# Isaac-McPadden/Farkle_II

Measured on AMD Instinct MI355X. Metric: simulated games/sec (whole node) at k=2, fixed strategy-grid size, higher is better.
Workload: dtype int32; 1 GPU; BASELINE configs[1]: k=2, 64-strategy grid, 10^7 games per GPU per step, root_seed 42, counts-only tallies; k=2, root_seed=42, parallelism=shuffle-range split x1, device=AMD Radeon Graphics, arch=gfx950:sramecc+:xnack-, compute_units=256, clock_mhz=2400

## Files before the change

farkle_ii_amd/backend.py:

```python
from __future__ import annotations

import ctypes as C
import os
import subprocess
from pathlib import Path

import numpy as np

from .strategies import STRATEGY_DTYPE

PKG_DIR = Path(__file__).resolve().parent
LIB_PATH = Path(os.environ.get("FARKLE_HIP_LIB", PKG_DIR / "libfarkle_hip.so"))
SRC_DIR = PKG_DIR / "csrc"
HIPCC = os.environ.get("HIPCC", "/opt/rocm/bin/hipcc")

COORD_DTYPE = np.dtype(
    [("purpose", "<u4"), ("pad", "<u4"), ("root_seed", "<u8"), ("k", "<u8"), ("shuffle_index", "<u8"),
     ("pair_id", "<u8"), ("order", "<u8"), ("game_index", "<u8"), ("seat_index", "<u8"), ("replicate_index", "<u8")]
)
OVERRIDE_DTYPE = np.dtype(
    [("root_seed", "<u8"), ("a", "<u8"), ("b", "<u8"), ("k_or_order", "<u4"), ("max_rounds", "<u4")]
)
SEAT_DTYPE = np.dtype(
    [("score", "<i4"), ("strategy", "<i4"), ("farkles", "<u2"), ("rolls", "<u2"), ("n_turns", "<u2"),
# ... 6 lines not shown
)
EVENT_DTYPE = np.dtype(
    [("dice", "<u4"), ("turn_score", "<i4"), ("points", "<u2"), ("round", "<u2"), ("seat", "u1"), ("used_left", "u1"),
     ("discards", "u1"), ("flags", "u1")]
)
TALLY_COLS = 26
LAG_COLS = 11
SEAT_STAT_COLS = 31
SEAT_RATIO_COLS = 4
SEAT_STAT_NAMES = ("exposures", "completed_exposures", "safety_limit_exposures", "wins", "final_score_sum", "final_score_square_sum",
                   "n_turns_sum", "n_turns_square_sum", "turn_round_mismatch_count", "turn_minus_rounds_sum",
                   "turn_minus_rounds_square_sum") + tuple(
    f"{name}_{kind}" for name in ("rank", "loss_margin", "rolls", "farkles", "highest_turn", "hot_dice", "smart_five_uses",
                                   "n_smart_five_dice", "smart_one_uses", "n_smart_one_dice") for kind in ("sum", "square_sum"))
COL_WINS, COL_ATTEMPTED, COL_COMPLETED, COL_SAFETY, COL_SUMS, COL_SQ_SUMS = 0, 1, 2, 3, 4, 15

FK_ERR_ROLL_LIMIT, FK_ERR_ARG, FK_ERR_COUNTER_OVERFLOW, FK_ERR_HIP, FK_ERR_NO_DEVICE, FK_ERR_COMM = -1, -2, -3, -4, -5, -6
COMM_ID_BYTES = 128


def row_dtype(k: int) -> np.dtype:
    return np.dtype([("n_rounds", "<u2"), ("status", "u1"), ("winner_seat", "i1"), ("seats", SEAT_DTYPE, (k,))])


class _DeviceInfo(C.Structure):
    _fields_ = [("name", C.c_char * 64), ("arch", C.c_char * 32), ("compute_units", C.c_int32), ("clock_mhz", C.c_int32),
                ("wavefront_size", C.c_int32), ("lds_bytes_per_cu", C.c_int32), ("hbm_bytes", C.c_uint64)]


class _Timing(C.Structure):
    _fields_ = [("perm_ms", C.c_float), ("seed_ms", C.c_float), ("play_ms", C.c_float), ("total_ms", C.c_float),
                ("play_launches", C.c_int32), ("play_block", C.c_int32), ("play_grid", C.c_int32),
                ("play_lds_bytes", C.c_int32), ("games", C.c_int64), ("prefetched_chunks", C.c_int32), ("play_clock_mhz", C.c_int32),
                ("play_block_end_p50_ms", C.c_float), ("play_block_end_max_ms", C.c_float), ("play_mixed_flags", C.c_int32)]


class FarkleHipError(RuntimeError):

    def __init__(self, code: int, message: str):
        super().__init__(message)
        self.code = code


def hip_sources() -> list[Path]:
    return [SRC_DIR / "farkle_hip.hip"]


VARIANTS = {"detour": ["-DFK_FORCE_DETOUR=4"]}


def library_path(variant: str | None = None) -> Path:
    return LIB_PATH if not variant else LIB_PATH.with_name(f"libfarkle_hip_{variant}.so")


def build_library(force: bool = False, verbose: bool = False, variant: str | None = None) -> Path:
    out = library_path(variant)
    deps = hip_sources() + [SRC_DIR / "fk_device.h", SRC_DIR / "fk_kernels.h", SRC_DIR / "fk_play_hc.h", SRC_DIR / "fk_shard_writer.h", SRC_DIR / "fk_perm_wave.h", SRC_DIR / "fk_row_columns_seats.h", SRC_DIR / "fk_matchups.h", SRC_DIR / "fk_game_stats.h", SRC_DIR / "fk_rare_events.h", SRC_DIR / "fk_bootstrap.h", SRC_DIR / "fk_root_stability.h", SRC_DIR / "fk_seat_analysis.h", SRC_DIR / "fk_trace.h", PKG_DIR.parent / "include" / "farkle_hip.h"]
    if out.exists() and not force and all(out.stat().st_mtime >= d.stat().st_mtime for d in deps):
        return out
    cmd = [HIPCC, "--offload-arch=gfx950", "-O3", "-std=c++17", "-fPIC", "-shared", *(VARIANTS[variant] if variant else []), "-o", str(out),
           *[str(s) for s in hip_sources()]]
    res = subprocess.run(cmd, capture_output=True, text=True)
    if verbose or res.returncode != 0:
        print(" ".join(cmd))
        print(res.stdout, res.stderr)
    if res.returncode != 0:
        raise RuntimeError(f"hipcc failed ({res.returncode}): {res.stderr[-2000:]}")
    return out


_EXPORTS = ["fk_init", "fk_destroy", "fk_last_error", "fk_get_device_info", "fk_get_timing", "fk_set_option",
            "fk_tournament_run", "fk_tournament_run_stats", "fk_tournament_run_all_player", "fk_tournament_run_game_stats", "fk_tournament_run_rare_events", "fk_tournament_run_lags", "fk_tournament_run_matchups", "fk_matchup_reduce", "fk_tournament_hint_next", "fk_play_games", "fk_h2h_run", "fk_h2h_run_blocks", "fk_coordinate_seeds", "fk_debug_score", "fk_debug_should_continue",
            "fk_debug_dice", "fk_debug_dice_state", "fk_debug_dice_keys", "fk_comm_unique_id", "fk_comm_init", "fk_reduce_tally", "fk_comm_destroy", "fk_tally_resident_reduce", "fk_comm_ranks", "fk_host_alloc", "fk_host_free", "fk_game_seeds",
            "fk_tournament_run_columns", "fk_row_columns_bytes", "fk_write_row_shards", "fk_debug_sha256", "fk_get_option", "fk_debug_deadline_handshake", "fk_debug_hold_memory", "fk_rows_wait", "fk_tournament_run_columns_seeds",
            "fk_last_play_instance", "fk_debug_bounded_draws", "fk_performance_bootstrap", "fk_root_stability_bootstrap", "fk_tournament_run_seat_counts", "fk_trace_games"]
_libs: dict = {}


def load_library(variant: str | None = None) -> C.CDLL:
    if variant not in _libs:
        path = library_path(variant)
        if not path.exists():
            raise FileNotFoundError(
                f"{path} is missing: build it with `python -c 'import __graft_entry__ as g; g.build()'` "
                "(there is no CPU fallback for the simulation path)")
        lib = C.CDLL(str(path))
        for name in _EXPORTS:
            getattr(lib, name)
        lib.fk_last_error.restype = C.c_char_p
        lib.fk_last_error.argtypes = [C.c_void_p]
        lib.fk_last_play_instance.restype = C.c_char_p
        lib.fk_last_play_instance.argtypes = [C.c_void_p]
        lib.fk_destroy.restype = None
# ... 691 lines not shown
```

farkle_ii_amd/csrc/farkle_hip.hip:

```cpp
#include "fk_kernels.h"
#include "fk_shard_writer.h"
#include "fk_perm_wave.h"
#include "fk_row_columns_seats.h"
#include "fk_matchups.h"
#include "fk_game_stats.h"
#include "fk_rare_events.h"
#include "fk_bootstrap.h"
#include "fk_root_stability.h"
#include "fk_seat_analysis.h"
#include "fk_trace.h"

#include <dlfcn.h>
#include <rccl/rccl.h>
#include <unistd.h>

#include <algorithm>
#include <atomic>
#include <chrono>
#include <cmath>
#include <memory>
#include <mutex>
#include <sys/mman.h>
#include <unordered_map>
#include <thread>
// ... 94 lines not shown
    const SeatReq *seats;
};

struct fk_ctx {
    int device = 0;
    hipStream_t stream = nullptr;
    hipStream_t prep_stream = nullptr;
    ChunkSet sets[2];
    int cur = 0;
    uint64_t table_epoch = 0;
    bool hint_valid = false;
    uint64_t hint_begin = 0, hint_end = 0;
    int32_t hint_state = 0, pipeline = 1;
    hipDeviceProp_t prop{};
    std::string err;
    fk_timing timing{};
    std::string play_instance;
    hipEvent_t ev[8] = {nullptr, nullptr, nullptr, nullptr, nullptr, nullptr, nullptr, nullptr};
    int32_t *err_host = nullptr;
    hipEvent_t main_idle = nullptr;
    struct PendingTimer {
        float *acc;
        hipEvent_t a, b;
    };
    std::vector<PendingTimer> pending;
    DevBuf strat, recs, rec0, tally, rows, ov, seatlist, coords, inv, slow, score_lut, discard_lut, block_out, stats, ratios, digest,
        dbg[6];
    std::vector<uint2> strat_host;
    int32_t longest_first = 1;
    int32_t blocks_per_cu = 0;
    int32_t max_waves = 6;
    int32_t lean = -1;
    int32_t gs = -1;
    int32_t uniform_flags_opt = -1;
    uint32_t table_flags = 0;
    uint32_t table_mixed_flags = 0xff00u;
    int64_t chunk_bytes = (int64_t)48 << 30;
    int32_t workspace_percent = 80;
    int64_t chunk_limit = 0;
    int64_t last_budget = 0;
    bool oom = false;
    std::vector<void *> hog;
    int32_t oom_replays = 0;
    int32_t batch_threshold = 0;
    int32_t use_lds_tally = -1;
    int32_t block = 0;
    int32_t hc = -1;
    int32_t hc_waves = 5;
    int32_t hc_block = 256;
    int32_t hc_tables = 1;
    int32_t hc_inc_regs = 1;
    int32_t hc_cl = -1;
    DevBuf lds_tables;
    DevBuf cold;
    int32_t clock_stamps = 0;
    DevBuf clk;
    int clk_grid = 0;
    DevBuf lag_v, lag_out, lag_lags, lag_edge, lag_tmp;
    DevBuf m_ids, m_dig, m_seat, m_rnd;
    DevBuf mr[36];
    uint64_t matchup_sort_mask = ~0ull;
    DevBuf g_rec, g_out;
    int64_t game_stats_window = 0;
    DevBuf r_sec, r_out, r_blk, r_base, r_head, r_seats;
    DevBuf sa_counts, sa[16];
    DevBuf tr[8];
// ... 615 lines not shown
    HIPCHK(c, hipGetLastError());
    return FK_OK;
}

size_t game_workspace_bytes(int32_t k, bool full_state, bool recs, bool rows) {
    return (size_t)k * ((full_state ? STATE_DW * 4 : 18) + 16) + 8 + (recs ? REC_DW * 4 + 4 : 0) +
           (rows ? sizeof(fk_row_hdr) + sizeof(fk_seat) * (size_t)k : 0);
}

int launch_play_stage(fk_ctx *c, const SeedArgs &sa, PlayArgs &pa, const LaunchPlan &plan, bool want_state, bool want_rec0, bool want_recs) {
    ChunkSet &cs = CSET(c);
    int rc;
    if (want_rec0) {
        rc = ensure(c, c->rec0, (size_t)sa.n_games * 4);
        if (rc) return rc;
    }
    if (want_recs) {
        rc = ensure(c, c->recs, (size_t)sa.n_games * REC_DW * 4);
        if (rc) return rc;
    }
    pa.sched = sa.sched;
    pa.seat_idx = sa.seat_idx;
    pa.state = sa.state;
    pa.state_dw = sa.state_dw;
    pa.inc = sa.inc;
    pa.rec0 = want_rec0 ? static_cast<uint32_t *>(c->rec0.p) : nullptr;
    pa.recs = want_recs ? static_cast<uint32_t *>(c->recs.p) : nullptr;
    pa.gs_out = (want_state && !plan.gs) ? 1u : 0u;
    pa.ticket = static_cast<uint32_t *>(cs.misc.p);
    pa.err = reinterpret_cast<int32_t *>(static_cast<uint8_t *>(cs.misc.p) + 16);
    const int auto_thr = sa.k >= 11 ? 16 : sa.k >= 9 ? 12 : 8;
    pa.batch_threshold = (uint32_t)std::max(1, std::min(64, c->batch_threshold > 0 ? c->batch_threshold : auto_thr));
    pa.use_lds_tally = plan.lds_tally ? 1u : 0u;
    pa.clk = nullptr;
    c->clk_grid = 0;
    if (c->clock_stamps) {
        const size_t bytes = (size_t)std::max(plan.grid, 1) * 4 * sizeof(unsigned long long);
        rc = ensure(c, c->clk, bytes);
        if (rc) return rc;
        HIPCHK(c, hipMemsetAsync(c->clk.p, 0, bytes, c->stream));
        pa.clk = static_cast<unsigned long long *>(c->clk.p);
    }
    {
        Timer t(c, &c->timing.play_ms, SLOT_PLAY);
        LaunchPlan lp = plan;
        lp.mixed_flags = (c->uniform_flags_opt != 0) ? c->table_mixed_flags : 0xff00u;
        pa.uflags = c->table_flags;
        hipError_t e = launch_play(lp, pa, c->stream);
        t.stop();
        HIPCHK(c, e);
        c->play_instance = lp.instance ? lp.instance : "";
        c->timing.play_grid = lp.launched_grid;
        c->timing.play_mixed_flags = lp.mixed_flags == MIXED_NONE ? (int32_t)MIXED_NONE
                                     : (lp.mixed_flags & ~MIXED_RB_FAV) == 0u ? (int32_t)MIXED_RB_FAV : (int32_t)MIXED_ALL;
        if (pa.clk) c->clk_grid = lp.launched_grid;
    }
    c->timing.play_launches += 1;
    c->timing.play_block = plan.block;
    c->timing.play_lds_bytes = (int32_t)plan.lds;
    c->timing.games += sa.n_games;
    return FK_OK;
}

int finish_timers(fk_ctx *c) {
    HIPCHK(c, collect_timers(c));
    if (c->clk_grid > 0) {
// ... 1 lines not shown
        HIPCHK(c, hipMemcpy(h.data(), c->clk.p, h.size() * sizeof(unsigned long long), hipMemcpyDeviceToHost));
        std::vector<double> mhz, ends;
        unsigned long long first = ~0ull;
        for (int b = 0; b < c->clk_grid; ++b) {
            const unsigned long long t0 = h[(size_t)b * 4], r0 = h[(size_t)b * 4 + 1], t1 = h[(size_t)b * 4 + 2], r1 = h[(size_t)b * 4 + 3];
            if (r1 > r0 && t1 > t0) {
                mhz.push_back(100.0 * (double)(t1 - t0) / (double)(r1 - r0));
                ends.push_back((double)r1);
                first = r0 < first ? r0 : first;
            }
        }
        if (!mhz.empty()) {
            std::nth_element(mhz.begin(), mhz.begin() + (std::ptrdiff_t)(mhz.size() / 2), mhz.end());
            c->timing.play_clock_mhz = (int32_t)(mhz[mhz.size() / 2] + 0.5);
            std::nth_element(ends.begin(), ends.begin() + (std::ptrdiff_t)(ends.size() / 2), ends.end());
            c->timing.play_block_end_p50_ms = (float)((ends[ends.size() / 2] - (double)first) * 1e-5);
            c->timing.play_block_end_max_ms = (float)((*std::max_element(ends.begin(), ends.end()) - (double)first) * 1e-5);
        }
        c->clk_grid = 0;
    }
    ChunkSet &cs = CSET(c);
    float ms = 0.f;
    if (hipEventElapsedTime(&ms, cs.ev[0], cs.ev[1]) == hipSuccess) c->timing.perm_ms += ms;
    if (cs.side) {
        c->timing.prefetched_chunks += 1;
    } else if (hipEventElapsedTime(&ms, cs.ev[2], cs.ev[3]) == hipSuccess) {
        c->timing.seed_ms += ms;
    }
    return FK_OK;
}

int finish_play(fk_ctx *c, const PlayArgs &pa, int64_t game_base, const char *what) {
    const int rc_dev = check_device_error(c, pa.err, game_base, what);
    const int rc = finish_timers(c);
    return rc_dev ? rc_dev : rc;
}

int run_chunk(fk_ctx *c, const SeedArgs &sa_in, PlayArgs pa, const LaunchPlan &plan, bool want_state, bool want_rec0, bool want_recs,
              int64_t game_base, const char *what) {
    SeedArgs sa = sa_in;
    ChunkSet &cs = CSET(c);
    cs.prepared = false;
    cs.side = false;
    HIPCHK(c, hipStreamWaitEvent(c->stream, cs.ready, 0));
    (void)hipEventRecord(cs.ev[0], c->stream);
    (void)hipEventRecord(cs.ev[1], c->stream);
    int rc = seed_stage(c, c->cur, c->stream, sa, plan.gs || want_state, true);
    if (rc) return rc;
    rc = launch_play_stage(c, sa, pa, plan, want_state, want_rec0, want_recs);
    if (rc) return rc;
    return finish_play(c, pa, game_base, what);
}

int prep_tournament_chunk(fk_ctx *c, int si, hipStream_t st_seed, const ChunkDesc &d, SeedArgs &sa) {
    ChunkSet &cs = c->sets[si];
    cs.prepared = false;
    hipStream_t st = c->stream;
    HIPCHK(c, hipStreamWaitEvent(st, cs.ready, 0));
    const int32_t S = (int32_t)d.S;
    const uint32_t n_sh = d.n_sh, slots = d.slots, gps = d.S / d.k;
    const uint32_t perm_blocks = (n_sh + slots - 1u) / slots;
    const SeedPool perm_prefix = seed_prefix(101u , d.root, (uint64_t)d.k);
    int rc = ensure(c, cs.perm, (size_t)perm_blocks * S * slots * 2);
    if (rc) return rc;
    (void)hipEventRecord(cs.ev[0], st);
    {
// ... 462 lines not shown
}

int fk_set_option(fk_ctx *c, const char *name, int64_t value) {
    if (!c || !name) return FK_ERR_ARG;
    std::string n(name);
    if (n == "chunk_bytes") c->chunk_bytes = std::max<int64_t>(value, 1 << 20);
    else if (n == "workspace_percent") c->workspace_percent = (int32_t)std::min<int64_t>(std::max<int64_t>(value, 1), 100000);
    else if (n == "comm_timeout_ms") {
        c->comm_timeout_ms = (int32_t)std::min<int64_t>(std::max<int64_t>(value, 0), 86400000);
        c->comm_timeout_set = true;
    }
    else if (n == "batch_threshold") c->batch_threshold = (int32_t)value;
    else if (n == "use_lds_tally") c->use_lds_tally = (int32_t)value;
    else if (n == "longest_first") c->longest_first = (int32_t)value;
    else if (n == "blocks_per_cu") c->blocks_per_cu = (int32_t)value;
    else if (n == "max_waves") c->max_waves = (int32_t)std::min<int64_t>(std::max<int64_t>(value, 1), 8);
    else if (n == "lean") c->lean = (int32_t)value;
    else if (n == "state_store") c->gs = (int32_t)value;
    else if (n == "rows_chunk_games") c->rows_chunk_games = std::max<int64_t>(value, 1);
    else if (n == "rows_async") c->rows_async = value != 0;
    else if (n == "resident_tally") {
        c->resident = value != 0;
        c->acc_n = 0;
    } else if (n == "hot_cold") {
        if (value != -1 && value != 0) return fail(c, FK_ERR_ARG, "hot_cold is -1 (auto: four and more seats) or 0 (never)");
        c->hc = (int32_t)value;
    }
    else if (n == "clock_stamps") c->clock_stamps = value != 0;
    else if (n == "perm_split") c->perm_split = (int32_t)value;
    else if (n == "perm_draw_wave") c->perm_draw_wave = (int32_t)value;
    else if (n == "columns_by_seat") c->columns_by_seat = (int32_t)value;
    else if (n == "pipeline") c->pipeline = (int32_t)value;
    else if (n == "uniform_flags") c->uniform_flags_opt = (int32_t)value;
    else if (n == "matchup_sort_key_mask") c->matchup_sort_mask = (uint64_t)value;
    else if (n == "game_stats_window") c->game_stats_window = std::max<int64_t>(value, 0);
    else if (n == "bootstrap_block") c->bootstrap_block = std::max<int64_t>(value, 0);
    else if (n == "block") {
        if (value != 0 && value != 64 && value != 128 && value != 256 && value != 512 && value != 768 && value != 1024)
            return fail(c, FK_ERR_ARG, "block must be 0, 64, 128, 256, 512, 768 (lean records only) or 1024");
        c->block = (int32_t)value;
    } else return fail(c, FK_ERR_ARG, "unknown option %s", name);
    return FK_OK;
}

int fk_rows_wait(fk_ctx *c, int32_t slot) {
    if (!c || slot < 0 || slot >= FK_ROWS_EVENTS) return FK_ERR_ARG;
    HIPCHK(c, hipSetDevice(c->device));
    HIPCHK(c, hipEventSynchronize(c->ev_call_copy[slot]));
    return FK_OK;
}

size_t fk_row_columns_bytes(int32_t k, int32_t games_per_shuffle) {
    return (k < 1 || games_per_shuffle < 1) ? 0 : fksw::shard_image_bytes(k, games_per_shuffle);
}

int fk_write_row_shards(const fk_shard_job *job, int64_t *byte_length, uint8_t *sha256, uint8_t *sidecar_sha256, char *error, size_t error_len) {
    auto say = [&](const std::string &m) {
        if (error && error_len) std::snprintf(error, error_len, "%s", m.c_str());
        return FK_ERR_ARG;
    };
    if (!job || !byte_length || !sha256) return say("job, byte_length and sha256 are required");
    if (!job->shuffle_index || !job->shuffle_seed || !job->batch_id || !job->game_seed || !job->columns || !job->directory || !job->footer_head ||
        !job->footer_kv || !job->footer_orders || !job->leaf_type || !job->leaf_paths)
        return say("a required field of the shard job is null");
    if ((job->side_body != nullptr) != (job->side_full != nullptr) || (job->side_body && (!job->side_directory || !sidecar_sha256)))
        return say("the sidecar template needs body, full, directory and a sidecar_sha256 output");
// ... 452 lines not shown
        pa.seat_strategy = nullptr;
        pa.tally = static_cast<unsigned long long *>(c->tally.p);
        pa.ov = static_cast<const DevOverride *>(c->ov.p);
        pa.n_ov = (uint32_t)dov.size();
        pa.mode = MODE_PERM;
        pa.n_games = n_games;
        pa.gps = gps;
        pa.n_sh = n_sh;
        pa.k = (uint32_t)k;
        pa.S = (uint32_t)S;
        pa.target50 = ceil_div50(target_score);
        pa.beat50 = floor_div50(target_score);
        pa.max_rounds = (uint32_t)max_rounds;
        pa.cold = static_cast<uint4 *>(c->cold.p);
        pa.lds_tables = static_cast<const uint8_t *>(c->lds_tables.p);

        HIPCHK(c, hipEventRecord(c->main_idle, c->stream));
        if (c->pipeline) {
            ChunkDesc next{};
            bool have_next = false;
            if (done + chunk_sh < n_sh_total) {
                next = describe(sh0 + n_sh, (uint32_t)std::min<uint64_t>(chunk_sh, n_sh_total - done - chunk_sh), state_dw);
                have_next = true;
            } else if (hinted) {
                next = describe(hint_begin, (uint32_t)std::min<uint64_t>(chunk_sh, hint_end - hint_begin), hint_dw);
                have_next = true;
            }
            if (have_next) {
                if ((rc = prep_tournament_chunk(c, c->cur ^ 1, c->prep_stream, next, c->sets[c->cur ^ 1].sa))) return rc;
            }
        }
        if (wait_ready) HIPCHK(c, hipStreamWaitEvent(c->stream, c->sets[c->cur].ready, 0));
        if ((rc = launch_play_stage(c, sa, pa, plan, want_state, want_recs || sq != nullptr, want_recs))) return rc;
        const bool defer_check = done + chunk_sh >= n_sh_total && !rows && c->err_host;
        if (defer_check) {
            HIPCHK(c, hipMemcpyAsync(c->err_host, pa.err, 2 * sizeof(int32_t), hipMemcpyDeviceToHost, c->stream));
            deferred = true;
            deferred_base = (int64_t)done * gps;
        } else {
            if ((rc = finish_play(c, pa, (int64_t)done * gps, "tournament"))) return rc;
        }
        const bool scheduled = c->longest_first != 0;
        if (want_state && scheduled) {
            if ((rc = ensure(c, c->inv, (size_t)n_games * 4))) return rc;
            hipLaunchKernelGGL(fk_invert_sched_kernel, dim3((n_games + 255u) / 256u), dim3(256), 0, c->stream,
                               static_cast<const uint32_t *>(CSET(c).order.p), n_games, static_cast<uint32_t *>(c->inv.p));
        }
        if (seat_stats || gst || sq) {
            rc = ensure(c, CSET(c).draws, (size_t)perm_blocks * S * slots * 2);
            if (rc) return rc;
            const uint32_t cells = perm_blocks * (uint32_t)S * slots;
            hipLaunchKernelGGL(fk_invert_perm_kernel, dim3((cells + 255u) / 256u), dim3(256), 0, c->stream,
                               static_cast<const uint16_t *>(CSET(c).perm.p), (uint32_t)S, slots, n_sh, static_cast<uint16_t *>(CSET(c).draws.p));
        }
        if (gst) {
            unsigned long long *o = static_cast<unsigned long long *>(c->g_out.p);
            const uint32_t rec_grid = std::max<uint32_t>(1u, std::min<uint32_t>((n_games + 255u) / 256u, 2048u));
            hipLaunchKernelGGL(fkg::fk_game_record_kernel, dim3(rec_grid), dim3(256), (size_t)(g_wr + g_wm + fkg::N_COUNTS) * 4, c->stream,
                               static_cast<const uint32_t *>(CSET(c).state.p), static_cast<const uint32_t *>(c->recs.p),
                               scheduled ? static_cast<const uint32_t *>(c->inv.p) : nullptr, n_games, gps, n_sh, (uint32_t)k, gst->rare_target,
                               g_wr, g_wm, static_cast<uint4 *>(c->g_rec.p), o + g_gc, o + g_gr, o + g_gru, g_spill);
            const uint32_t want_seg = std::max<uint32_t>(1u, (2048u + (uint32_t)S - 1u) / (uint32_t)S);
            const uint32_t rows_per_seg = std::max<uint32_t>(256u, (n_sh + want_seg - 1u) / want_seg);
            const uint32_t n_seg = (n_sh + rows_per_seg - 1u) / rows_per_seg;
            hipLaunchKernelGGL(fkg::fk_game_stats_gather_kernel, dim3((uint32_t)S, n_seg), dim3(256), (size_t)(g_wr + 2 * g_wm + fkg::N_COUNTS) * 4,
                               c->stream, static_cast<const uint4 *>(c->g_rec.p), static_cast<const uint16_t *>(CSET(c).draws.p), slots,
                               (uint32_t)S, (uint32_t)k, gps, n_sh, rows_per_seg, g_wr, g_wm, g_rb, g_mb, o + g_sc, o + g_sr, o + g_sru, o + g_ssp,
// ... 1548 lines not shown
```

farkle_ii_amd/csrc/fk_device.h:

```cpp
#pragma once

#include <hip/hip_runtime.h>
#include <stdint.h>

namespace fk {

constexpr uint32_t SS_INIT_A = 0x43b0d7e5u, SS_MULT_A = 0x931e8875u;
constexpr uint32_t SS_INIT_B = 0x8b51f9ddu, SS_MULT_B = 0x58f38dedu;
constexpr uint32_t SS_MIX_L = 0xca01f9ddu, SS_MIX_R = 0x4973f715u;

__host__ __device__ constexpr uint32_t ss_hc(int c) {
    uint32_t h = SS_INIT_A;
    for (int i = 0; i < c; ++i) h *= SS_MULT_A;
    return h;
}

__host__ __device__ inline uint32_t ss_hashmix(uint32_t v, uint32_t &hc) {
    v ^= hc;
    hc *= SS_MULT_A;
    v *= hc;
    v ^= v >> 16;
    return v;
}

// ... 853 lines not shown
}

template <bool LEAN, uint32_t MIXED = 0xffffu>
__host__ __device__ inline bool roll_back_end50w(uint32_t e, uint32_t x, uint32_t n, const Strat50 &sp, uint32_t uniform_bits, bool final_round,
                                                 int32_t stb50, RollRegs &r, bool &overflow) {
    const int32_t score50 = (int32_t)(e & 63u) - (int32_t)((x >> DW_POINTS_SHIFT) & 0xffu);
    const uint32_t used = ((e >> 6) & 7u) - (x >> DW_DICE_SHIFT);
    return roll_back_end50_core<LEAN, MIXED>(score50, used, x & DW_INC, (x >> DW_D1_SHIFT) & DW_INC, n, sp, uniform_bits, final_round, stb50, r, overflow);
}

struct Table2 {
    uint32_t seat, rounds, trigger, final_round, safety;
    int32_t score_to_beat;
};
struct Advance2 {
    bool ended, sw;
};
__host__ __device__ inline Advance2 advance2_table50(bool over, int32_t score, int32_t target50, uint32_t max_rounds, Table2 &t) {
    const bool fr = t.final_round != 0u;
    const bool trig = over & !fr & (score >= target50);
    const bool close = over & !fr & !trig & (t.seat != 0u);
    const bool last = close & (t.rounds >= max_rounds);
    const bool ended = last | (over & fr);
    t.rounds += (close & !last) ? 1u : 0u;
    t.safety = last ? 1u : t.safety;
    t.score_to_beat = trig ? score : t.score_to_beat;
    t.trigger = trig ? t.seat : t.trigger;
    t.final_round = (fr | trig) ? 1u : 0u;
    const bool sw = over & !ended;
    t.seat ^= sw ? 1u : 0u;
    return Advance2{ended, sw};
}

}
```

farkle_ii_amd/csrc/fk_kernels.h:

```cpp
#pragma once

#include "../../include/farkle_hip.h"
#include "fk_device.h"

#include <hip/hip_runtime.h>

using namespace fk;

namespace {

constexpr uint32_t HC_AFTER_6_WORDS = ss_hc(24);
constexpr uint32_t HC_AFTER_12_WORDS = ss_hc(48);
constexpr uint32_t HC_AFTER_14_WORDS = ss_hc(56);

enum : uint32_t { MODE_PERM = 0, MODE_LIST = 1, MODE_BLOCKS = 2 };

enum : uint32_t {
    F_LO0 = 0, F_LO1, F_HI0, F_HI1, F_INC_LO0, F_INC_LO1, F_INC_HI0, F_INC_HI1,
    F_BUF, F_SCORE, F_CA, F_CB, F_CC, F_CD, F_CE, F_SPX, F_SPY, NF
};
constexpr uint32_t CE_HAS_BUF_SHIFT = 17, CE_HAS_SCORED = 1u << 16, CE_HAS_BUF = 1u << CE_HAS_BUF_SHIFT;
static_assert(CE_HAS_SCORED == BE_HAS_SCORED, "fk_device.h's roll back end sets the flag in cE");
constexpr uint32_t CE_IDX_SHIFT = 18;
constexpr uint32_t LEAN_DW = 10;
constexpr int32_t LEAN_MAX_TARGET50 = 64000;

enum : uint32_t { R_LO0 = 0, R_LO1, R_HI0, R_HI1, R_BUF, R_SCORE, R_CA, R_CB, R_CC, R_CD, R_CE, R_IDX, STATE_DW = 12 };

constexpr uint32_t REC_DW = 8, REC_SAFETY = 0x80000000u;

constexpr uint32_t LT_COLS = 24;
constexpr uint32_t TICKET_CHUNK = 64;

struct DevOverride {
    uint32_t game;
    uint32_t max_rounds;
};

// ... 29 lines not shown
};

struct PlayArgs {
    const uint2 *strat;
    const uint32_t *score_lut;
    const uint8_t *discard_lut;
    const uint16_t *perm_T;
    uint32_t perm_slots;
    const int32_t *seat_strategy;
    const uint32_t *game_block;
    uint32_t *state;
    uint32_t state_dw;
    const uint4 *inc;
    const uint16_t *seat_idx;
    const uint32_t *sched;
    unsigned long long *tally;
    uint32_t *rec0;
    uint32_t *recs;
    uint32_t gs_out;
    uint32_t *ticket;
    int32_t *err;
    const DevOverride *ov;
    uint32_t n_ov;
    uint32_t mode;
    uint32_t n_games, gps, n_sh, k, S;
    int32_t target50;
    int32_t beat50;
    uint32_t max_rounds;
    uint32_t batch_threshold;
    uint32_t use_lds_tally;
    uint32_t uflags;
    uint4 *cold;
    const uint8_t *lds_tables;
    unsigned long long *clk;
};

__device__ inline void clock_stamp(unsigned long long *clk, uint32_t which) {
    if (!clk) return;
    unsigned long long *slot = clk + (size_t)blockIdx.x * 4u + 2u * which;
    if (which == 0u) {
        if (threadIdx.x == 0) {
            slot[0] = __builtin_amdgcn_s_memtime();
            slot[1] = __builtin_amdgcn_s_memrealtime();
        }
    } else if ((threadIdx.x & 63u) == 0u) {
        atomicMax(slot, (unsigned long long)__builtin_amdgcn_s_memtime());
        atomicMax(slot + 1, (unsigned long long)__builtin_amdgcn_s_memrealtime());
    }
}

__device__ inline uint32_t lane_id() { return threadIdx.x & 63u; }

__device__ inline uint32_t mbcnt(uint64_t mask) {
    return __builtin_amdgcn_mbcnt_hi((uint32_t)(mask >> 32), __builtin_amdgcn_mbcnt_lo((uint32_t)mask, 0u));
}

__device__ inline Strat unpack_strat(uint2 v) { return Strat{(int32_t)v.x, v.y}; }

__device__ inline uint32_t perm_at(const uint16_t *perm, uint32_t S, uint32_t slots, uint32_t sh, uint32_t e) {
    const uint32_t b = sh / slots, l = sh - b * slots;
    return perm[((size_t)b * S + e) * slots + l];
}

constexpr int PERM_BLOCK = 512, PERM_WAVES = PERM_BLOCK / 64;

__global__ __launch_bounds__(PERM_BLOCK) void fk_perm_kernel(SeedPool prefix, uint64_t shuffle0, uint32_t n_sh, uint32_t S,
// ... 853 lines not shown
                g[0] = make_uint4((uint32_t)rng.lo, (uint32_t)(rng.lo >> 32), (uint32_t)rng.hi, (uint32_t)(rng.hi >> 32));
                g[1] = make_uint4(rng.buf, (uint32_t)score, cA, (cB & 0xffffu) | (own_turns << 16));
                uint32_t *g2 = reinterpret_cast<uint32_t *>(g + 2);
                g2[0] = cC;
                g2[1] = cD;
                g2[2] = (cB >> 16) | (cE & (CE_HAS_SCORED | CE_HAS_BUF));
                advance(score);
                return;
            }
        }
        if (LEAN) {
            rec[0] = make_uint2((uint32_t)rng.lo, (uint32_t)(rng.lo >> 32));
            rec[1] = make_uint2((uint32_t)rng.hi, (uint32_t)(rng.hi >> 32));
            rec[2] = make_uint2(rng.buf, cA);
            rec[3] = make_uint2(cB, cC);
            rec[4] = make_uint2(cD, cE);
        } else {
            L(F_LO0, s) = (uint32_t)rng.lo;
            L(F_LO1, s) = (uint32_t)(rng.lo >> 32);
            L(F_HI0, s) = (uint32_t)rng.hi;
            L(F_HI1, s) = (uint32_t)(rng.hi >> 32);
            L(F_BUF, s) = rng.buf;
            L(F_SCORE, s) = (uint32_t)score;
            L(F_CA, s) = cA;
            L(F_CB, s) = cB;
            L(F_CC, s) = cC;
            L(F_CD, s) = cD;
            L(F_CE, s) = cE;
        }
        if (PK2) advance2(over, score);
        else if (!GS && over) advance(score);
    };

    auto handover = [&](uint64_t waiting) {
        const bool mine = (st == ST_FRESH || st == ST_ENDED);
        if (st == ST_ENDED) finish_game();
        const uint32_t n = (uint32_t)__popcll(waiting);
        const uint32_t avail = pool_end - pool_next;
        uint32_t new_base = 0, new_avail = 0;
        if (avail < n && !exhausted) {
            const uint32_t first = (uint32_t)__builtin_amdgcn_readfirstlane(__ffsll((long long)waiting) - 1);
            uint32_t base = 0;
            if (mine && lane_id() == first) base = atomicAdd(a.ticket, TICKET_CHUNK);
            base = (uint32_t)__builtin_amdgcn_readlane((int)base, (int)first);
            if (base >= a.n_games) {
                exhausted = 1;
            } else {
                new_base = base;
                new_avail = min(TICKET_CHUNK, a.n_games - base);
                if (new_avail < TICKET_CHUNK) exhausted = 1;
            }
        }
        if (mine) {
            const uint32_t rank = mbcnt(waiting);
            uint32_t ticket = 0xffffffffu;
            if (rank < avail) ticket = pool_next + rank;
            else if (rank - avail < new_avail) ticket = new_base + (rank - avail);
            if (ticket != 0xffffffffu) init_game(a.sched ? a.sched[ticket] : ticket, ticket);
            else st = ST_DONE;
        }
        if (n <= avail) {
            pool_next += n;
        } else {
            const uint32_t used_new = min(n - avail, new_avail);
            pool_next = new_base + used_new;
            pool_end = new_base + new_avail;
        }
    };

    auto handover_due = [&](uint64_t waiting, uint64_t active) -> bool {
        return waiting && (!active || (uint32_t)__popcll(waiting) >= a.batch_threshold || exhausted);
    };
    while (true) {
        uint64_t waiting = __ballot(st == ST_FRESH || st == ST_ENDED);
        uint64_t active = __ballot(st == ST_ACTIVE);
        if (!(waiting | active)) break;
        if (handover_due(waiting, active)) {
            handover(waiting);
            continue;
        }
        bool playing = st == ST_ACTIVE;
        do {
            if (playing) roll_step();
            playing = st == ST_ACTIVE;
            waiting = __ballot(st == ST_ENDED);
            active = __ballot(playing);
        } while (active && !handover_due(waiting, active));
    }

    if (a.use_lds_tally) {
        __syncthreads();
        for (uint32_t i = tid; i < a.S * LT_COLS; i += BLOCK) {
            const unsigned long long v = tl[i];
            if (v == 0ull) continue;
            const uint32_t idx = i / LT_COLS, c = i - idx * LT_COLS;
            if (c == LT_COLS - 1u) continue;
            const uint32_t col = (c == 0u) ? 0u : (c == 1u) ? 2u : (c == 2u) ? 3u : (c < 13u) ? (c + 1u) : (c + 2u);
            atomicAdd(&a.tally[(size_t)idx * FK_TALLY_COLS + col], v);
        }
    }
    clock_stamp(a.clk, 1u);
}

#include "fk_play_hc.h"

constexpr uint32_t LAG_WIN_BIT = 0x8000u;

__global__ __launch_bounds__(256) void fk_lag_values_kernel(const uint32_t *recs, const uint16_t *perm_T, uint32_t perm_slots, uint32_t S,
                                                            uint32_t k, uint32_t gps, uint32_t n_games, uint16_t *V) {
    const size_t t = (size_t)blockIdx.x * blockDim.x + threadIdx.x;
    if (t >= (size_t)n_games * k) return;
    const uint32_t id = (uint32_t)(t / k), seat = (uint32_t)(t - (size_t)id * k);
    const uint32_t sh = id / gps, g = id - sh * gps;
    const uint4 q0 = *reinterpret_cast<const uint4 *>(recs + (size_t)id * REC_DW);
    const bool won = !(q0.x & REC_SAFETY) && ((q0.x >> 24) & 0x7fu) == seat;
    const uint32_t idx = perm_at(perm_T, S, perm_slots, sh, g * k + seat);
    V[(size_t)sh * S + idx] = (uint16_t)((q0.z & 0x7fffu) | (won ? LAG_WIN_BIT : 0u));
}

__global__ __launch_bounds__(256) void fk_lag_sums_kernel(const uint16_t *V, uint32_t S, uint32_t valid_from, uint32_t first_row, uint32_t n_rows,
                                                          uint32_t rows_per_seg, const int32_t *lags, uint32_t n_lags, long long *out) {
    const uint32_t s = blockIdx.x * blockDim.x + threadIdx.x;
    if (s >= S) return;
    const uint32_t r0 = first_row + blockIdx.y * rows_per_seg, r1 = min(r0 + rows_per_seg, n_rows);
    for (uint32_t li = 0; li < n_lags; ++li) {
        const uint32_t lag = (uint32_t)lags[li];
        long long n = 0, wx = 0, wy = 0, wxy = 0, rx = 0, ry = 0, rxx = 0, ryy = 0, rxy = 0;
        for (uint32_t r = max(r0, valid_from + lag); r < r1; ++r) {
            const uint32_t later = V[(size_t)r * S + s], earlier = V[(size_t)(r - lag) * S + s];
            const long long a = earlier & 0x7fffu, b = later & 0x7fffu, wa = earlier >> 15, wb = later >> 15;
            n += 1;
            wx += wa, wy += wb, wxy += wa & wb;
            rx += a, ry += b, rxx += a * a, ryy += b * b, rxy += a * b;
// ... 550 lines not shown
```

include/farkle_hip.h:

```cpp
#ifndef FARKLE_HIP_H
#define FARKLE_HIP_H

#include <stddef.h>
#include <stdint.h>

#ifdef __cplusplus
extern "C" {
#endif

enum {
    FK_OK = 0,
    FK_ERR_ROLL_LIMIT = -1,
    FK_ERR_ARG = -2,
    FK_ERR_COUNTER_OVERFLOW = -3,
    FK_ERR_HIP = -4,
    FK_ERR_NO_DEVICE = -5,
    FK_ERR_COMM = -6,
    FK_ERR_IO = -7
};

enum { FK_COMPLETED = 0, FK_SAFETY_LIMIT = 1 };

typedef struct {
    int32_t score_threshold;
// ... 29 lines not shown
    uint32_t purpose;
    uint32_t pad;
    uint64_t root_seed, k, shuffle_index, pair_id, order, game_index, seat_index, replicate_index;
} fk_coord;

#define FK_MAX_PLAYERS 128
#define FK_SEAT_STAT_COLS 31
#define FK_LAG_COLS 11
#define FK_MAX_LAGS 16
#define FK_TALLY_COLS 26

typedef struct {
    char name[64];
    char arch[32];
    int32_t compute_units;
    int32_t clock_mhz;
    int32_t wavefront_size;
    int32_t lds_bytes_per_cu;
    uint64_t hbm_bytes;
} fk_device_info;

typedef struct {
    float perm_ms;
    float seed_ms;
    float play_ms;
    float total_ms;
    int32_t play_launches;
    int32_t play_block, play_grid, play_lds_bytes;
    int64_t games;
    int32_t prefetched_chunks;
    int32_t play_clock_mhz;
    float play_block_end_p50_ms, play_block_end_max_ms;
    int32_t play_mixed_flags;
} fk_timing;

typedef struct fk_ctx fk_ctx;

int fk_init(int device_ordinal, fk_ctx **out);
void fk_destroy(fk_ctx *ctx);
const char *fk_last_error(fk_ctx *ctx);
int fk_get_device_info(fk_ctx *ctx, fk_device_info *out);
int fk_get_timing(fk_ctx *ctx, fk_timing *out);
const char *fk_last_play_instance(fk_ctx *ctx);
int fk_host_alloc(fk_ctx *ctx, size_t bytes, void **out);
int fk_host_free(fk_ctx *ctx, void *p);
int fk_set_option(fk_ctx *ctx, const char *name, int64_t value);
int fk_get_option(fk_ctx *ctx, const char *name, int64_t *value);

int fk_tournament_run(fk_ctx *ctx, const fk_strategy *strategies, int32_t S, int32_t k, uint64_t root_seed,
                      uint64_t shuffle_begin, uint64_t shuffle_end, uint32_t shuffles_per_batch,
                      int32_t target_score, int32_t max_rounds, const fk_override *ov, int32_t n_ov,
                      int64_t *tally, void *rows, int32_t *perms);

int fk_tournament_run_columns(fk_ctx *ctx, const fk_strategy *strategies, int32_t S, int32_t k, uint64_t root_seed,
                              uint64_t shuffle_begin, uint64_t shuffle_end, uint32_t shuffles_per_batch,
                              int32_t target_score, int32_t max_rounds, const fk_override *ov, int32_t n_ov,
                              int64_t *tally, const int32_t *strategy_ids, void *columns);
int fk_tournament_run_columns_seeds(fk_ctx *ctx, const fk_strategy *strategies, int32_t S, int32_t k, uint64_t root_seed,
                                    uint64_t shuffle_begin, uint64_t shuffle_end, uint32_t shuffles_per_batch, int32_t target_score,
                                    int32_t max_rounds, const fk_override *overrides, int32_t n_overrides, int64_t *tally,
                                    const int32_t *strategy_ids, void *columns, uint32_t *shuffle_seeds, uint32_t *game_seeds);
size_t fk_row_columns_bytes(int32_t k, int32_t games_per_shuffle);
int fk_rows_wait(fk_ctx *ctx, int32_t slot);

typedef struct {
    int32_t k, games_per_shuffle, n_shuffles, threads, atomic, rng_purpose_namespace;
// ... 160 lines not shown
```

Baseline: 1.208 billion games/s.

## Add flat k=2 handover path with scalar-register bases and specialized finish

Adds a specialized handover path for two-player games without blocking. Game init and finish use precomputed uniform base addresses held in scalar registers and a feature bitmask, plus a branch-light winner selection (finish2_50). This targets the per-game setup and teardown cost in the wave-level handover loop, which the old path paid through generic init_game/finish_game calls. The new path is on by default and can be turned off with the flat_handover option. A compile-time handover counting variant is also added for profiling; its extra output fields enlarge the timing struct.

```diff
diff --git a/farkle_ii_amd/backend.py b/farkle_ii_amd/backend.py
--- a/farkle_ii_amd/backend.py
+++ b/farkle_ii_amd/backend.py
@@ -62,7 +62,9 @@
     _fields_ = [("perm_ms", C.c_float), ("seed_ms", C.c_float), ("play_ms", C.c_float), ("total_ms", C.c_float),
                 ("play_launches", C.c_int32), ("play_block", C.c_int32), ("play_grid", C.c_int32),
                 ("play_lds_bytes", C.c_int32), ("games", C.c_int64), ("prefetched_chunks", C.c_int32), ("play_clock_mhz", C.c_int32),
-                ("play_block_end_p50_ms", C.c_float), ("play_block_end_max_ms", C.c_float), ("play_mixed_flags", C.c_int32)]
+                ("play_block_end_p50_ms", C.c_float), ("play_block_end_max_ms", C.c_float), ("play_mixed_flags", C.c_int32),
+                ("ho_handovers", C.c_int64), ("ho_lanes_served", C.c_int64), ("ho_trips", C.c_int64),
+                ("ho_waiting_lane_trips", C.c_int64), ("ho_rolling_lane_trips", C.c_int64), ("ho_waves", C.c_int64)]
 
 
 class FarkleHipError(RuntimeError):
@@ -77,6 +79,7 @@
 
 
 VARIANTS = {"detour": ["-DFK_FORCE_DETOUR=4"]}
+TOOL_VARIANTS = {"count": ["-DFK_COUNT_HANDOVER"]}
 
 
 def library_path(variant: str | None = None) -> Path:
@@ -88,7 +91,7 @@
     deps = hip_sources() + [SRC_DIR / "fk_device.h", SRC_DIR / "fk_kernels.h", SRC_DIR / "fk_play_hc.h", SRC_DIR / "fk_shard_writer.h", SRC_DIR / "fk_perm_wave.h", SRC_DIR / "fk_row_columns_seats.h", SRC_DIR / "fk_matchups.h", SRC_DIR / "fk_game_stats.h", SRC_DIR / "fk_rare_events.h", SRC_DIR / "fk_bootstrap.h", SRC_DIR / "fk_root_stability.h", SRC_DIR / "fk_seat_analysis.h", SRC_DIR / "fk_trace.h", PKG_DIR.parent / "include" / "farkle_hip.h"]
     if out.exists() and not force and all(out.stat().st_mtime >= d.stat().st_mtime for d in deps):
         return out
-    cmd = [HIPCC, "--offload-arch=gfx950", "-O3", "-std=c++17", "-fPIC", "-shared", *(VARIANTS[variant] if variant else []), "-o", str(out),
+    cmd = [HIPCC, "--offload-arch=gfx950", "-O3", "-std=c++17", "-fPIC", "-shared", *({**VARIANTS, **TOOL_VARIANTS}[variant] if variant else []), "-o", str(out),
            *[str(s) for s in hip_sources()]]
     res = subprocess.run(cmd, capture_output=True, text=True)
     if verbose or res.returncode != 0:
diff --git a/farkle_ii_amd/csrc/farkle_hip.hip b/farkle_ii_amd/csrc/farkle_hip.hip
--- a/farkle_ii_amd/csrc/farkle_hip.hip
+++ b/farkle_ii_amd/csrc/farkle_hip.hip
@@ -150,6 +150,7 @@
     int32_t max_waves = 6;
     int32_t lean = -1;
     int32_t gs = -1;
+    int32_t flat_handover = 1;
     int32_t uniform_flags_opt = -1;
     uint32_t table_flags = 0;
     uint32_t table_mixed_flags = 0xff00u;
@@ -831,6 +832,12 @@
     const int auto_thr = sa.k >= 11 ? 16 : sa.k >= 9 ? 12 : 8;
     pa.batch_threshold = (uint32_t)std::max(1, std::min(64, c->batch_threshold > 0 ? c->batch_threshold : auto_thr));
     pa.use_lds_tally = plan.lds_tally ? 1u : 0u;
+    pa.no_flat = c->flat_handover ? 0u : 1u;
+#ifdef FK_COUNT_HANDOVER
+    pa.hcount = reinterpret_cast<unsigned long long *>(static_cast<uint8_t *>(cs.misc.p) + 128);
+#else
+    pa.hcount = nullptr;
+#endif
     pa.clk = nullptr;
     c->clk_grid = 0;
     if (c->clock_stamps) {
@@ -898,6 +905,12 @@
 
 int finish_play(fk_ctx *c, const PlayArgs &pa, int64_t game_base, const char *what) {
     const int rc_dev = check_device_error(c, pa.err, game_base, what);
+    if (pa.hcount) {
+        unsigned long long h[6] = {0, 0, 0, 0, 0, 0};
+        HIPCHK(c, hipMemcpy(h, pa.hcount, sizeof(h), hipMemcpyDeviceToHost));
+        c->timing.ho_handovers += (int64_t)h[0], c->timing.ho_lanes_served += (int64_t)h[1], c->timing.ho_trips += (int64_t)h[2];
+        c->timing.ho_waiting_lane_trips += (int64_t)h[3], c->timing.ho_rolling_lane_trips += (int64_t)h[4], c->timing.ho_waves += (int64_t)h[5];
+    }
     const int rc = finish_timers(c);
     return rc_dev ? rc_dev : rc;
 }
@@ -1426,6 +1439,7 @@
     else if (n == "columns_by_seat") c->columns_by_seat = (int32_t)value;
     else if (n == "pipeline") c->pipeline = (int32_t)value;
     else if (n == "uniform_flags") c->uniform_flags_opt = (int32_t)value;
+    else if (n == "flat_handover") c->flat_handover = value != 0 ? 1 : 0;
     else if (n == "matchup_sort_key_mask") c->matchup_sort_mask = (uint64_t)value;
     else if (n == "game_stats_window") c->game_stats_window = std::max<int64_t>(value, 0);
     else if (n == "bootstrap_block") c->bootstrap_block = std::max<int64_t>(value, 0);
@@ -1944,7 +1958,7 @@
         }
         if (wait_ready) HIPCHK(c, hipStreamWaitEvent(c->stream, c->sets[c->cur].ready, 0));
         if ((rc = launch_play_stage(c, sa, pa, plan, want_state, want_recs || sq != nullptr, want_recs))) return rc;
-        const bool defer_check = done + chunk_sh >= n_sh_total && !rows && c->err_host;
+        const bool defer_check = done + chunk_sh >= n_sh_total && !rows && c->err_host && !pa.hcount;
         if (defer_check) {
             HIPCHK(c, hipMemcpyAsync(c->err_host, pa.err, 2 * sizeof(int32_t), hipMemcpyDeviceToHost, c->stream));
             deferred = true;
diff --git a/farkle_ii_amd/csrc/fk_device.h b/farkle_ii_amd/csrc/fk_device.h
--- a/farkle_ii_amd/csrc/fk_device.h
+++ b/farkle_ii_amd/csrc/fk_device.h
@@ -909,4 +909,51 @@
     return Advance2{ended, sw};
 }
 
-}
+constexpr uint32_t LEAN_IDX_SHIFT = 18;
+struct LeanCounters {
+    uint32_t cA, cB, cC, cD, cE;
+};
+struct Finish2 {
+    bool completed;
+    uint32_t winner, widx;
+    uint32_t m[10];
+};
+
+__host__ __device__ inline Finish2 finish2_50_decoded(const LeanCounters &s0, const LeanCounters &s1, uint32_t rounds, uint32_t final_round,
+                                                      uint32_t max_rounds) {
+    const LeanCounters *seats[2] = {&s0, &s1};
+    uint32_t score[2], idx[2], farkles[2], rolls[2], highest[2], sf_uses[2], sf_dice[2], so_uses[2], so_dice[2], hot[2];
+    for (int s = 0; s < 2; ++s) {
+        const LeanCounters &r = *seats[s];
+        score[s] = r.cE & 0xffffu, idx[s] = r.cE >> LEAN_IDX_SHIFT;
+        rolls[s] = r.cA & 0xffffu, farkles[s] = r.cA >> 16;
+        highest[s] = r.cB & 0xffffu, hot[s] = r.cB >> 16;
+        sf_uses[s] = r.cC & 0xffffu, sf_dice[s] = r.cC >> 16;
+        so_uses[s] = r.cD & 0xffffu, so_dice[s] = r.cD >> 16;
+    }
+    Finish2 f;
+    f.completed = max_rounds != 0u && final_round != 0u;
+    f.winner = score[1] > score[0] ? 1u : 0u;
+    const uint32_t w = f.winner;
+    f.widx = idx[w];
+    f.m[0] = score[w] * 50u, f.m[1] = rounds, f.m[2] = farkles[w], f.m[3] = rolls[w], f.m[4] = highest[w] * 50u;
+    f.m[5] = sf_uses[w], f.m[6] = sf_dice[w], f.m[7] = so_uses[w], f.m[8] = so_dice[w], f.m[9] = hot[w];
+    return f;
+}
+
+__host__ __device__ inline Finish2 finish2_50(const LeanCounters &s0, const LeanCounters &s1, uint32_t rounds, uint32_t final_round,
+                                              uint32_t max_rounds) {
+    (void)max_rounds;
+    const bool second = (s1.cE & 0xffffu) > (s0.cE & 0xffffu);
+    const uint32_t a = second ? s1.cA : s0.cA, b = second ? s1.cB : s0.cB, c = second ? s1.cC : s0.cC, d = second ? s1.cD : s0.cD,
+                   e = second ? s1.cE : s0.cE;
+    Finish2 f;
+    f.completed = final_round != 0u;
+    f.winner = second ? 1u : 0u;
+    f.widx = e >> LEAN_IDX_SHIFT;
+    f.m[0] = (e & 0xffffu) * 50u, f.m[1] = rounds, f.m[2] = a >> 16, f.m[3] = a & 0xffffu, f.m[4] = (b & 0xffffu) * 50u;
+    f.m[5] = c & 0xffffu, f.m[6] = c >> 16, f.m[7] = d & 0xffffu, f.m[8] = d >> 16, f.m[9] = b >> 16;
+    return f;
+}
+
+}
diff --git a/farkle_ii_amd/csrc/fk_kernels.h b/farkle_ii_amd/csrc/fk_kernels.h
--- a/farkle_ii_amd/csrc/fk_kernels.h
+++ b/farkle_ii_amd/csrc/fk_kernels.h
@@ -4,6 +4,8 @@
 #include "fk_device.h"
 
 #include <hip/hip_runtime.h>
+
+#include <type_traits>
 
 using namespace fk;
 
@@ -99,6 +101,8 @@
     uint32_t uflags;
     uint4 *cold;
     const uint8_t *lds_tables;
+    uint32_t no_flat;
+    unsigned long long *hcount;
     unsigned long long *clk;
 };
 
@@ -1018,9 +1022,153 @@
         else if (!GS && over) advance(score);
     };
 
-    auto handover = [&](uint64_t waiting) {
+    constexpr bool FLAT2 = PK2 && !BLK;
+    static_assert(CE_IDX_SHIFT == LEAN_IDX_SHIFT, "finish2_50 reads the strategy index of a lean record");
+    enum : uint32_t { HO_LDS_TALLY = 1, HO_REC0 = 2, HO_RECS = 4, HO_GS_OUT = 8, HO_OV = 16, HO_SCHED = 32, HO_PERM = 64, HO_IDX_STATE = 128,
+                      HO_FLAT = 256 };
+    typedef uint32_t u32x2 __attribute__((ext_vector_type(2)));
+    typedef __attribute__((address_space(1))) u32x4 global_u4_rw;
+    typedef const __attribute__((address_space(1))) u32x2 global_u2;
+    typedef __attribute__((address_space(1))) uint32_t global_u32;
+    uint32_t ho_bits = 0, st_rec = 0, ho_max_rounds = a.max_rounds, ho_thr = a.batch_threshold;
+    int32_t ho_beat50 = a.beat50;
+    uint64_t st_base = 0, inc_base = 0, idx_base = 0, sched_base = 0, strat_base = 0, rec0_base = 0;
+    if constexpr (FLAT2) {
+        const bool idx_state = a.state_dw == STATE_DW;
+        const bool flat = !a.no_flat && (idx_state || a.seat_idx != nullptr) && (uint64_t)a.n_games * (2u * STATE_DW * 4u) <= 0xffffffffull;
+        ho_bits = (a.use_lds_tally ? HO_LDS_TALLY : 0u) | (a.rec0 ? HO_REC0 : 0u) | (a.recs ? HO_RECS : 0u) | (a.gs_out ? HO_GS_OUT : 0u) |
+             (a.n_ov ? HO_OV : 0u) | (a.sched ? HO_SCHED : 0u) | (a.mode == MODE_PERM ? HO_PERM : 0u) | (idx_state ? HO_IDX_STATE : 0u) |
+             (flat ? HO_FLAT : 0u);
+        st_rec = a.state_dw * 4u;
+        st_base = (uint64_t)(uintptr_t)a.state, inc_base = (uint64_t)(uintptr_t)a.inc, sched_base = (uint64_t)(uintptr_t)a.sched;
+        idx_base = idx_state ? st_base + R_IDX * 4u : (uint64_t)(uintptr_t)a.seat_idx;
+        strat_base = (uint64_t)(uintptr_t)a.strat, rec0_base = (uint64_t)(uintptr_t)a.rec0;
+        asm volatile("" : "+s"(ho_bits), "+s"(st_rec), "+s"(ho_max_rounds), "+s"(ho_thr), "+s"(ho_beat50), "+s"(st_base), "+s"(inc_base), "+s"(idx_base),
+                     "+s"(sched_base), "+s"(strat_base), "+s"(rec0_base));
+    }
+    auto ld1 = [](uint64_t base, uint32_t off) __attribute__((always_inline)) -> uint32_t { return *(const global_u32 *)(base + (uint64_t)off); };
+    auto ld2 = [](uint64_t base, uint32_t off) __attribute__((always_inline)) -> u32x2 { return *(global_u2 *)(base + (uint64_t)off); };
+    auto ld4 = [](uint64_t base, uint32_t off) __attribute__((always_inline)) -> u32x4 { return *(global_u4 *)(base + (uint64_t)off); };
+
+    auto init_game2 = [&](uint32_t ticket) __attribute__((always_inline)) {
+        uint32_t ho = ho_bits;
+        asm volatile("" : "+s"(ho));
+        uint32_t id = ticket, slot = ticket;
+        uint32_t id_ld = 0;
+        if (ho & HO_SCHED) {
+            id_ld = ld1(sched_base, ticket * 4u);
+        } else if (ho & HO_PERM) {
+            const uint32_t sh = id / a.gps, g = id - sh * a.gps;
+            slot = g * a.n_sh + sh;
+        }
+        const uint32_t soff = slot * (2u * st_rec);
+        const u32x4 s0 = ld4(st_base, soff), s1 = ld4(st_base, soff + st_rec);
+        const u32x4 inc = ld4(inc_base, slot * 32u);
+        const uint32_t ioff = (ho & HO_IDX_STATE) ? soff : slot * 4u;
+        const uint32_t w0 = ld1(idx_base, ioff), w1 = ld1(idx_base, ioff + ((ho & HO_IDX_STATE) ? st_rec : 0u));
+        if (ho & HO_SCHED) id = id_ld;
+        const uint32_t idx0 = (ho & HO_IDX_STATE) ? w0 : (w0 & 0xffffu), idx1 = (ho & HO_IDX_STATE) ? w1 : (w1 >> 16);
+        u32x2 pk0 = ld2(strat_base, idx0 * 8u), pk1 = ld2(strat_base, idx1 * 8u);
+        game_id = id;
+        seed_slot = slot;
+        max_rounds = ho_max_rounds;
+        if (ho & HO_OV) {
+            uint32_t lo = 0, hi = a.n_ov;
+            while (lo < hi) {
+                const uint32_t mid = (lo + hi) >> 1;
+                if (a.ov[mid].game < id) lo = mid + 1u;
+                else hi = mid;
+            }
+            if (lo < a.n_ov && a.ov[lo].game == id) max_rounds = a.ov[lo].max_rounds;
+        }
+        uint2 *r0 = reinterpret_cast<uint2 *>(lds + lane_base), *r1 = reinterpret_cast<uint2 *>(lds + SEAT_STRIDE + lane_base);
+        r0[0] = make_uint2(s0.x, s0.y), r0[1] = make_uint2(s0.z, s0.w);
+        r0[2] = make_uint2(0u, 0u), r0[3] = make_uint2(0u, 0u), r0[4] = make_uint2(0u, idx0 << CE_IDX_SHIFT);
+        r1[0] = make_uint2(s1.x, s1.y), r1[1] = make_uint2(s1.z, s1.w);
+        r1[2] = make_uint2(0u, 0u), r1[3] = make_uint2(0u, 0u), r1[4] = make_uint2(0u, idx1 << CE_IDX_SHIFT);
+        pk0.y = (pk0.y & 0xff00u) | ((uint32_t)(int32_t)(int8_t)(pk0.y & 0xffu) << 16);
+        pk1.y = (pk1.y & 0xff00u) | ((uint32_t)(int32_t)(int8_t)(pk1.y & 0xffu) << 16);
+        pk_seat0 = make_uint2(pk0.x, pk0.y);
+        pk_delta = make_uint2(pk0.x ^ pk1.x, pk0.y ^ pk1.y);
+        seat = 0;
+        final_round = 0;
+        score_to_beat = ho_beat50;
+        own_inc_lo = (uint64_t)inc.x | ((uint64_t)inc.y << 32);
+        own_inc_hi = (uint64_t)inc.z | ((uint64_t)inc.w << 32);
+        own_thr = (int32_t)pk0.x;
+        own_bits = pk0.y;
+        own_rec = lds_addr(lane_base);
+        own_inc_at = inc_base + (uint64_t)(slot * 32u);
+        dice = 6;
+        turn_score = 0;
+        rolls_this_turn = 0;
+        const bool none = max_rounds == 0u;
+        rounds = none ? 0u : 1u;
+        st = none ? (uint32_t)ST_ENDED : (uint32_t)ST_ACTIVE;
+    };
+
+    auto finish_game2 = [&]() __attribute__((always_inline)) {
+        uint32_t ho = ho_bits;
+        asm volatile("" : "+s"(ho));
+        const uint2 *r0 = reinterpret_cast<const uint2 *>(lds + lane_base), *r1 = reinterpret_cast<const uint2 *>(lds + SEAT_STRIDE + lane_base);
+        const uint2 p2 = r0[2], p3 = r0[3], p4 = r0[4], q2 = r1[2], q3 = r1[3], q4 = r1[4];
+        const LeanCounters c0{p2.y, p3.x, p3.y, p4.x, p4.y}, c1{q2.y, q3.x, q3.y, q4.x, q4.y};
+        const Finish2 f = finish2_50(c0, c1, rounds, final_round, max_rounds);
+        const uint32_t idx0 = c0.cE >> CE_IDX_SHIFT, idx1 = c1.cE >> CE_IDX_SHIFT, widx = f.widx;
+        if (ho & HO_GS_OUT) {
+            const uint32_t last = (max_rounds != 0u && own_rec != lds_addr(lane_base)) ? 1u : 0u;
+            const uint32_t t0 = rounds + ((final_round != 0u && last == 0u) ? 1u : 0u), t1 = rounds;
+            const uint2 p0 = r0[0], p1 = r0[1], q0 = r1[0], q1 = r1[1];
+            const uint32_t soff = seed_slot * (2u * st_rec);
+            global_u4_rw *g0 = (global_u4_rw *)(st_base + (uint64_t)soff), *g1 = (global_u4_rw *)(st_base + (uint64_t)(soff + st_rec));
+            g0[0] = u32x4{p0.x, p0.y, p1.x, p1.y};
+            g0[1] = u32x4{p2.x, c0.cE & 0xffffu, c0.cA, (c0.cB & 0xffffu) | (t0 << 16)};
+            g0[2] = u32x4{c0.cC, c0.cD, (c0.cB >> 16) | (c0.cE & (CE_HAS_SCORED | CE_HAS_BUF)), idx0};
+            g1[0] = u32x4{q0.x, q0.y, q1.x, q1.y};
+            g1[1] = u32x4{q2.x, c1.cE & 0xffffu, c1.cA, (c1.cB & 0xffffu) | (t1 << 16)};
+            g1[2] = u32x4{c1.cC, c1.cD, (c1.cB >> 16) | (c1.cE & (CE_HAS_SCORED | CE_HAS_BUF)), idx1};
+        }
+        if (ho & HO_LDS_TALLY) {
+            if (!f.completed || !(ho & HO_PERM)) {
+                const uint32_t col = f.completed ? 1u : 2u;
+                atomicAdd(&tl[idx0 * LT_COLS + col], 1ull);
+                atomicAdd(&tl[idx1 * LT_COLS + col], 1ull);
+            }
+            if (f.completed) {
+                unsigned long long *t = tl + widx * LT_COLS;
+                atomicAdd(&t[0], 1ull);
+#pragma unroll
+                for (int j = 0; j < 10; ++j) {
+                    atomicAdd(&t[3 + j], (unsigned long long)f.m[j]);
+                    atomicAdd(&t[13 + j], (unsigned long long)f.m[j] * f.m[j]);
+                }
+            }
+        }
+        if (ho & HO_REC0) {
+            const uint32_t d0 = f.completed ? (widx | (f.winner << 24)) : REC_SAFETY;
+            *(global_u32 *)(rec0_base + (uint64_t)(game_id * 4u)) = d0;
+            if (ho & HO_RECS) {
+                uint32_t m[10];
+#pragma unroll
+                for (int j = 0; j < 10; ++j) m[j] = f.completed ? f.m[j] : 0u;
+                uint4 *r = reinterpret_cast<uint4 *>(a.recs + (size_t)game_id * REC_DW);
+                r[0] = make_uint4(d0, m[0], rounds | (m[2] << 16), m[3] | (m[4] << 16));
+                r[1] = make_uint4(m[5] | (m[6] << 16), m[7] | (m[8] << 16), m[9], 0u);
+            }
+        }
+    };
+
+#ifdef FK_COUNT_HANDOVER
+    uint32_t cnt_handovers = 0, cnt_served = 0, cnt_trips = 0, cnt_waiting = 0, cnt_rolling = 0;
+#endif
+
+    auto handover = [&](uint64_t waiting, auto flat) {
+        constexpr bool FLAT = decltype(flat)::value;
         const bool mine = (st == ST_FRESH || st == ST_ENDED);
-        if (st == ST_ENDED) finish_game();
+        if (st == ST_ENDED) {
+            if constexpr (FLAT) finish_game2();
+            else finish_game();
+        }
         const uint32_t n = (uint32_t)__popcll(waiting);
         const uint32_t avail = pool_end - pool_next;
         uint32_t new_base = 0, new_avail = 0;
@@ -1042,8 +1190,12 @@
             uint32_t ticket = 0xffffffffu;
             if (rank < avail) ticket = pool_next + rank;
             else if (rank - avail < new_avail) ticket = new_base + (rank - avail);
-            if (ticket != 0xffffffffu) init_game(a.sched ? a.sched[ticket] : ticket, ticket);
-            else st = ST_DONE;
+            if (ticket != 0xffffffffu) {
+                if constexpr (FLAT) init_game2(ticket);
+                else init_game(a.sched ? a.sched[ticket] : ticket, ticket);
+            } else {
+                st = ST_DONE;
+            }
         }
         if (n <= avail) {
             pool_next += n;
@@ -1055,23 +1207,37 @@
     };
 
     auto handover_due = [&](uint64_t waiting, uint64_t active) -> bool {
-        return waiting && (!active || (uint32_t)__popcll(waiting) >= a.batch_threshold || exhausted);
-    };
-    while (true) {
-        uint64_t waiting = __ballot(st == ST_FRESH || st == ST_ENDED);
-        uint64_t active = __ballot(st == ST_ACTIVE);
-        if (!(waiting | active)) break;
-        if (handover_due(waiting, active)) {
-            handover(waiting);
-            continue;
-        }
-        bool playing = st == ST_ACTIVE;
-        do {
-            if (playing) roll_step();
-            playing = st == ST_ACTIVE;
-            waiting = __ballot(st == ST_ENDED);
-            active = __ballot(playing);
-        } while (active && !handover_due(waiting, active));
+        return waiting && (!active || (uint32_t)__popcll(waiting) >= ho_thr || exhausted);
+    };
+    auto play = [&](auto flat) {
+        while (true) {
+            uint64_t waiting = __ballot(st == ST_FRESH || st == ST_ENDED);
+            uint64_t active = __ballot(st == ST_ACTIVE);
+            if (!(waiting | active)) break;
+            if (handover_due(waiting, active)) {
+#ifdef FK_COUNT_HANDOVER
+                cnt_handovers += 1u, cnt_served += (uint32_t)__popcll(waiting);
+#endif
+                handover(waiting, flat);
+                continue;
+            }
+            bool playing = st == ST_ACTIVE;
+            do {
+#ifdef FK_COUNT_HANDOVER
+                cnt_trips += 1u, cnt_waiting += (uint32_t)__popcll(waiting), cnt_rolling += (uint32_t)__popcll(active);
+#endif
+                if (playing) roll_step();
+                playing = st == ST_ACTIVE;
+                waiting = __ballot(st == ST_ENDED);
+                active = __ballot(playing);
+            } while (active && !handover_due(waiting, active));
+        }
+    };
+    if constexpr (FLAT2) {
+        if (ho_bits & HO_FLAT) play(std::true_type{});
+        else play(std::false_type{});
+    } else {
+        play(std::false_type{});
     }
 
     if (a.use_lds_tally) {
@@ -1085,6 +1251,12 @@
             atomicAdd(&a.tally[(size_t)idx * FK_TALLY_COLS + col], v);
         }
     }
+#ifdef FK_COUNT_HANDOVER
+    if (a.hcount && lane_id() == 0u) {
+        const uint32_t c[6] = {cnt_handovers, cnt_served, cnt_trips, cnt_waiting, cnt_rolling, 1u};
+        for (int i = 0; i < 6; ++i) atomicAdd(&a.hcount[i], (unsigned long long)c[i]);
+    }
+#endif
     clock_stamp(a.clk, 1u);
 }
 
diff --git a/include/farkle_hip.h b/include/farkle_hip.h
--- a/include/farkle_hip.h
+++ b/include/farkle_hip.h
@@ -85,6 +85,7 @@
     int32_t play_clock_mhz;
     float play_block_end_p50_ms, play_block_end_max_ms;
     int32_t play_mixed_flags;
+    int64_t ho_handovers, ho_lanes_served, ho_trips, ho_waiting_lane_trips, ho_rolling_lane_trips, ho_waves;
 } fk_timing;
 
 typedef struct fk_ctx fk_ctx;
```

Result: faster. 1.244 billion games/s, median of 6 (+2.9%).
